# sml2004/CUDA-powered-mesh-handling-and-Iterative-solvers

Measured on NVIDIA B200. Metric: cg_iters_per_s, higher is better.
Workload: dtype f64

## Files before the change

### cuda-powered-mesh-handling-and-iterative-solvers_b200/csrc/dist.cu

```cuda
#include <cstdlib>

#include "spmv_dev.cuh"

namespace femb {

constexpr int MAXP = 16;
constexpr long long SPIN_TIMEOUT_CYCLES = 4000000000ll;

struct SymHeader {
  volatile long long flagA[MAXP];
  volatile long long flagB[MAXP];
  volatile long long flagC[MAXP];
  volatile double redB[MAXP];
  volatile double redC[MAXP];
  volatile double red2[2][4][MAXP];
  double pad[MAXP];
  volatile unsigned long long ll[2][MAXP][8];
  volatile long long flagS[MAXP];
  long long pad2[MAXP];
};
static_assert(sizeof(SymHeader) % 256 == 0, "header keeps p 256-byte aligned");

struct DistState {
  double rs_old, rs_new, pAp, alpha, beta;
// ... 967 lines not shown
    FEMB_CUDA(cudaLaunchCooperativeKernel(kern, dim3(G), dim3(SPMV_THREADS), kargs, 0, s));
    FEMB_CUDA(cudaEventRecord(pev[1], s));
    FEMB_CUDA(cudaMemcpyAsync(hfin, st, sizeof(DistState), cudaMemcpyDeviceToHost, s));
    FEMB_CUDA(cudaStreamSynchronize(s));
    float pms = 0.f;
    cudaEventElapsedTime(&pms, pev[0], pev[1]);
    if (hfin->status == 3 || hfin->stop == 3) {
      set_error("distributed CG: timed out waiting for a peer rank (flag never arrived)");
      return FEMB_ERR_NCCL;
    }
    result_host->iterations = hfin->iterations;
    result_host->status = hfin->status;
    result_host->rs = hfin->rs_new;
    result_host->loop_ms = pms;
    result_host->index_bytes = 4;
    return FEMB_OK;
  }
  if (bptr != nullptr && nnbr > 0 && n_interior > 0 && !getenv("FEMB_DIST_SEPARATE_PUSH")) dist_push_kernel<<<gp, 256, 0, s>>>(pe, send_idx, st);
  cudaGraph_t graph = nullptr;
  cudaGraphExec_t exec = nullptr;
  FEMB_CUDA(cudaStreamBeginCapture(s, cudaStreamCaptureModeThreadLocal));
  const bool folded = bptr != nullptr && nnbr > 0 && n_interior > 0 && !getenv("FEMB_DIST_SEPARATE_PUSH");
  BoundaryPush bp{folded ? bptr : nullptr, bk, boff, n_interior};
  static const bool classic_env = getenv("FEMB_DIST_CLASSIC") != nullptr;
  const bool classic = classic_env && block == 1 && !minv;
  const bool pdl = pdl_enabled() && !classic;
  const long long pin = classic ? 0 : spmv_pin_entries(nnz);
  static const int vec_waves = getenv("FEMB_DIST_VEC_WAVES") ? atoi(getenv("FEMB_DIST_VEC_WAVES")) : 8;
  const int g2m = pdl ? grid_for(n, DV_THREADS, vec_waves) : g2;
  for (int k = 0; k < check_every; ++k) {
// ... 50 lines not shown
  }
  float ms = 0.f;
  if (rc == FEMB_OK) cudaEventElapsedTime(&ms, tev[0], tev[1]);
  cudaGraphExecDestroy(exec);
  cudaGraphDestroy(graph);
  if (rc != FEMB_OK) return rc;
  if (fin->status == 3) {
    set_error("distributed CG: timed out waiting for a peer rank (flag never arrived)");
    return FEMB_ERR_NCCL;
  }
  result_host->iterations = fin->stop ? fin->iterations : max_iter;
  result_host->status = fin->stop ? fin->status : 2;
  result_host->rs = fin->rs_new;
  result_host->loop_ms = ms;
  result_host->index_bytes = 4;
  if (trace && fin->it > 20) {
    static long long h[TRACE_ITERS * 12];
    cudaMemcpy(h, trace, sizeof(h), cudaMemcpyDeviceToHost);
    const int i1 = std::min(fin->it, TRACE_ITERS) - 2;
    double acc[8] = {0, 0, 0, 0, 0, 0, 0, 0};
    for (int i = 10; i < i1; ++i) {
      const long long* t = h + i * 12;
      if (classic) {
        acc[0] += t[1] - t[0];
        acc[1] += t[3] - t[2];
        acc[2] += t[4] - t[3];
        acc[3] += t[6] - t[5];
        acc[4] += t[7] - t[6];
        acc[5] += t[9] - t[8];
        acc[6] += t[10] - t[9];
// ... 22 lines not shown
```

### cuda-powered-mesh-handling-and-iterative-solvers_b200/csrc/krylov.cu

```cuda
#include <cstdlib>

#include "spmv_dev.cuh"

namespace femb {

struct CGState {
  double rs_old, rs_new, pAp, alpha, beta;
  int it, stop, status, iterations;
  unsigned int ticket1, ticket2;
  int fin, fin_status;
};

template <int THREADS>
__device__ __forceinline__ void cg_k1_epilogue_n(double dot, double* __restrict__ partial, CGState* __restrict__ st, double eps, int guards) {
  const double t = block_sum<THREADS>(dot);
  __shared__ bool last;
  if (threadIdx.x == 0) {
    partial[blockIdx.x] = t;
    __threadfence();
    last = atomicAdd(&st->ticket1, 1u) == gridDim.x - 1;
  }
  __syncthreads();
  if (last) {
    __threadfence();
// ... 129 lines not shown
      st ? &st->stop : nullptr, pin, wvec);
  if (st && st->stop) return;
  if (FUSED) {
    if (rvec) cg_k1_epilogue3_n<TMA_THREADS>(dot, extra[0], extra[1], partial, st, eps, guards & 1, tol);
    else cg_k1_epilogue_n<TMA_THREADS>(dot, partial, st, eps, guards & 1);
  }
}

template <bool FUSED>
__global__ void __launch_bounds__(TMA_THREADS) spmv_tma16_kernel(long long n, long long nnz, const int* __restrict__ crow, const int* __restrict__ col,
                                                                 const double* __restrict__ val, const double* __restrict__ x,
                                                                 double* __restrict__ y, const unsigned char* __restrict__ mask,
                                                                 double* __restrict__ partial, CGState* __restrict__ st, double eps, int guards,
                                                                 const double* __restrict__ rvec, double tol, long long pin,
                                                                 const double* __restrict__ wvec, const unsigned short* __restrict__ col16,
                                                                 const unsigned char* __restrict__ tile_ok) {
  pdl_launch_dependents();
  double extra[2] = {0.0, 0.0};
  const double dot = spmv_tma16_rows<TMA16_STAGES, TMA16_CAP>(n, nnz, crow, col, col16, tile_ok, val, x, y, mask, (guards & 2) != 0, FUSED, rvec,
                                                             rvec ? extra : nullptr, st ? &st->stop : nullptr, pin, wvec);
  if (st && st->stop) return;
  if (FUSED) {
    if (rvec) cg_k1_epilogue3_n<TMA_THREADS>(dot, extra[0], extra[1], partial, st, eps, guards & 1, tol);
    else cg_k1_epilogue_n<TMA_THREADS>(dot, partial, st, eps, guards & 1);
  }
}

__global__ void __launch_bounds__(TMA_THREADS) idx16_encode_kernel(long long n, const int* __restrict__ crow, const int* __restrict__ col,
                                                                   unsigned short* __restrict__ col16, unsigned char* __restrict__ tile_ok,
                                                                   int* __restrict__ bad) {
  const long long ntiles = (n + TMA_THREADS - 1) / TMA_THREADS;
  for (long long t = blockIdx.x; t < ntiles; t += gridDim.x) {
    const long long r = t * TMA_THREADS + threadIdx.x;
    bool ok = true;
    if (r < n) {
      const int a = __ldg(crow + r), b = __ldg(crow + r + 1);
      long long prev = r;
      for (int j = a; j < b; ++j) {
        const long long c = __ldg(col + j), d = j == a ? prev - c : c - prev;
        ok = ok && d >= (j == a ? 0 : 1) && d <= 65535;
        col16[j] = (unsigned short)d;
        prev = c;
      }
    }
    ok = __syncthreads_and(ok);
    if (threadIdx.x == 0) {
      tile_ok[t] = ok ? 1 : 0;
      if (!ok) atomicAdd(bad, 1);
    }
  }
}

template <int LR, bool FUSED>
__global__ void __launch_bounds__(TMA_THREADS) spmv_bsr3_tma_kernel(long long nb, long long nnzb, const int* __restrict__ brow,
                                                                    const int* __restrict__ bcol, const double* __restrict__ bval,
                                                                    const double* __restrict__ x, double* __restrict__ y,
                                                                    const unsigned char* __restrict__ mask, double* __restrict__ partial,
                                                                    CGState* __restrict__ st, double eps, int guards,
                                                                    const double* __restrict__ rvec, double tol, const double* __restrict__ wvec) {
  if (st && st->stop) return;
  const double dot = spmv_bsr3_tma_rows<LR, true>(nb, nnzb, brow, bcol, bval, x, y, mask, (guards & 2) != 0, FUSED);
  if (FUSED) cg_k1_epilogue_n<TMA_THREADS>(dot, partial, st, eps, guards & 1);
}

// ... 253 lines not shown
  const double avg = n > 0 ? (double)nnz / (double)n : 1.0;
  static const bool force_vector = getenv("FEMB_SPMV_VECTOR") != nullptr, force_stream = getenv("FEMB_SPMV_STREAM") != nullptr;
  if (force_vector) return -(avg <= 3 ? 2 : avg <= 6 ? 4 : avg <= 24 ? 8 : avg <= 48 ? 16 : 32);
  static const bool force_tma = getenv("FEMB_SPMV_TMA") != nullptr;
  if (!force_stream && !force_tma && avg >= 64.0) return -32;
  if (!force_stream) return 100 + tma_pick_lr(n, nnz);
  for (int lr = 1; lr <= 32; lr *= 2)
    if ((SPMV_THREADS / lr) * avg * 1.25 <= STREAM_CAP) return lr;
  return 32;
}

static thread_local long long nnz_hint = 0;
static thread_local bool pdl_hint = false;
static thread_local long long pin_hint = 0;
static thread_local const unsigned short* col16_hint = nullptr;
static thread_local const unsigned char* tile_ok_hint = nullptr;

template <bool FUSED>
static void launch_spmv(int lanes, int grid, cudaStream_t s, long long n, const int* crow, const int* col, const double* val, const double* x,
                        double* y, const unsigned char* mask, double* partial, CGState* st, double eps, int guards,
                        const double* rvec = nullptr, double tol = 0.0, const double* wvec = nullptr) {
#define FEMB_SPMV_ARGS n, crow, col, val, x, y, mask, partial, st, eps, guards, rvec, tol, wvec
#define FEMB_TMA(LRV)                                                                                                              \
  {                                                                                                                                \
    cudaFuncSetAttribute(spmv_tma_kernel<LRV, FUSED>, cudaFuncAttributeMaxDynamicSharedMemorySize, (int)TMA_SMEM);                 \
    launch_pdl(spmv_tma_kernel<LRV, FUSED>, grid, TMA_THREADS, TMA_SMEM, s, pdl_hint, n, nnz_hint, crow, col, val, x, y, mask, partial, st, eps, \
               guards, rvec, tol, pin_hint, wvec);                                                                               \
  }
#define FEMB_BSR(LRV)                                                                                                              \
  {                                                                                                                                \
    cudaFuncSetAttribute(spmv_bsr3_tma_kernel<LRV, FUSED>, cudaFuncAttributeMaxDynamicSharedMemorySize, (int)BSR_SMEM);            \
// ... 7 lines not shown
    else                                                                                                                           \
      spmv_bsr3_vec_kernel<FUSED, UV, false><<<grid, BSRV_THREADS, 0, s>>>(n / 3, nnz_hint, crow, col, val, x, y, mask, partial, st, eps, guards, rvec, tol, wvec); \
  }
    case 300: FEMB_BSRV(4) break;
    case 301: FEMB_BSRV(2) break;
    case 201: FEMB_BSR(1) break;
    case 202: FEMB_BSR(2) break;
    case 204: FEMB_BSR(4) break;
    case 208: FEMB_BSR(8) break;
    case 216: FEMB_BSR(16) break;
    case 232: FEMB_BSR(32) break;
    case 101:
      if (col16_hint) {
        cudaFuncSetAttribute(spmv_tma16_kernel<FUSED>, cudaFuncAttributeMaxDynamicSharedMemorySize, (int)TMA16_SMEM);
        launch_pdl(spmv_tma16_kernel<FUSED>, grid, TMA_THREADS, TMA16_SMEM, s, pdl_hint, n, nnz_hint, crow, col, val, x, y, mask, partial, st,
                   eps, guards, rvec, tol, pin_hint, wvec, col16_hint, tile_ok_hint);
      } else {
        FEMB_TMA(1)
      }
      break;
    case 102: FEMB_TMA(2) break;
    case 104: FEMB_TMA(4) break;
    case 108: FEMB_TMA(8) break;
    case 116: FEMB_TMA(16) break;
    case 132: FEMB_TMA(32) break;
    case 1: spmv_stream_kernel<1, FUSED><<<grid, SPMV_THREADS, 0, s>>>(FEMB_SPMV_ARGS); break;
    case 2: spmv_stream_kernel<2, FUSED><<<grid, SPMV_THREADS, 0, s>>>(FEMB_SPMV_ARGS); break;
    case 4: spmv_stream_kernel<4, FUSED><<<grid, SPMV_THREADS, 0, s>>>(FEMB_SPMV_ARGS); break;
    case 8: spmv_stream_kernel<8, FUSED><<<grid, SPMV_THREADS, 0, s>>>(FEMB_SPMV_ARGS); break;
    case 16: spmv_stream_kernel<16, FUSED><<<grid, SPMV_THREADS, 0, s>>>(FEMB_SPMV_ARGS); break;
    case 32: spmv_stream_kernel<32, FUSED><<<grid, SPMV_THREADS, 0, s>>>(FEMB_SPMV_ARGS); break;
// ... 76 lines not shown
  SolveCtx* ctx = solve_ctx(as_stream(stream));
  if (!ctx) return FEMB_ERR_CUDA;
  cudaStream_t s = ctx->stream;
  const int guards = minv ? 0 : 1;
  if (minv) eps = 0.0;
  double *r = work, *p = work + n, *Ap = work + 2 * n;
  int lanes[8], g1[8], gmax = 1;
  for (int m = 0; m < nmat; ++m) lanes[m] = pick_lanes(n, mats[m].nnz, mats[m].block);
  static const bool classic_env = getenv("FEMB_CG_CLASSIC") != nullptr;
  const int ll = lanes[nmat - 1];
  static const bool bsr_merged = getenv("FEMB_BSR_MERGED") != nullptr;
  const bool merged = !classic_env && ((ll >= 300 && bsr_merged) || (ll >= 100 && ll < 200) || ll < 0);
  static const bool idx32_env = getenv("FEMB_SPMV_IDX32") != nullptr;
  bool use16 = !idx32_env && merged && nmat == 1 && lanes[0] == 101 && max_iter >= 16;
  const long long ntiles16 = (n + TMA_THREADS - 1) / TMA_THREADS;
  const size_t flags_off = 256, col16_off = flags_off + (((size_t)ntiles16 + 255) & ~(size_t)255);
  if (use16) {
    const size_t need16 = col16_off + 2 * (((size_t)mats[0].nnz + 7) & ~(size_t)7);
    if (ctx->idx16_bytes < need16) {
      if (ctx->graph_exec) cudaGraphExecDestroy(ctx->graph_exec), ctx->graph_exec = nullptr, ctx->graph_key_bytes = 0;
      FEMB_CUDA(cudaStreamSynchronize(s));
      if (ctx->idx16) cudaFree(ctx->idx16);
      ctx->idx16 = nullptr, ctx->idx16_bytes = 0;
      if (cudaMalloc(&ctx->idx16, need16) == cudaSuccess) ctx->idx16_bytes = need16;
      else ctx->idx16 = nullptr, use16 = false, cudaGetLastError();
    }
  }
  if (use16) {
    unsigned char* base16 = static_cast<unsigned char*>(ctx->idx16);
    static_assert(2 * sizeof(CGState) + sizeof(int) <= 512 && 512 + sizeof(int) <= SOLVE_PINNED_BYTES, "pinned status buffer");
    int* bad_host = reinterpret_cast<int*>(static_cast<unsigned char*>(ctx->pinned) + 512);
    FEMB_CUDA(cudaMemsetAsync(base16, 0, sizeof(int), s));
    idx16_encode_kernel<<<(int)std::min<long long>(ntiles16, (long long)SMS * 16), TMA_THREADS, 0, s>>>(
        n, mats[0].crow, mats[0].col, reinterpret_cast<unsigned short*>(base16 + col16_off), base16 + flags_off, reinterpret_cast<int*>(base16));
    FEMB_LAUNCH_CHECK();
    FEMB_CUDA(cudaMemcpyAsync(bad_host, base16, sizeof(int), cudaMemcpyDeviceToHost, s));
    FEMB_CUDA(cudaStreamSynchronize(s));
    use16 = (long long)*bad_host * 100 <= ntiles16;
  }
  const unsigned short* col16 = use16 ? reinterpret_cast<const unsigned short*>(static_cast<unsigned char*>(ctx->idx16) + col16_off) : nullptr;
  const unsigned char* tile_ok = use16 ? static_cast<unsigned char*>(ctx->idx16) + flags_off : nullptr;
  for (int m = 0; m < nmat; ++m) {
    g1[m] = spmv_grid(n, lanes[m], merged && m == nmat - 1);
    if (use16) g1[m] = tma16_grid(n);
    gmax = std::max(gmax, g1[m]);
  }
  const int g2 = grid_for(n, VEC_THREADS, 8);
  static const int vec_waves = getenv("FEMB_VEC_WAVES") ? atoi(getenv("FEMB_VEC_WAVES")) : 8;
  const int g2v = grid_for(n, VEC_THREADS, vec_waves);
  const size_t need = 256 + sizeof(double) * (size_t)std::max(3 * gmax, g2);
  if (ctx->dev_scratch_bytes < need) {
    if (ctx->graph_exec) cudaGraphExecDestroy(ctx->graph_exec), ctx->graph_exec = nullptr, ctx->graph_key_bytes = 0;
    FEMB_CUDA(cudaStreamSynchronize(s));
    if (ctx->dev_scratch) cudaFree(ctx->dev_scratch);
    ctx->dev_scratch = nullptr, ctx->dev_scratch_bytes = 0;
    FEMB_CUDA(cudaMalloc(&ctx->dev_scratch, need + need / 2));
    ctx->dev_scratch_bytes = need + need / 2;
  }
  static_assert(sizeof(CGState) <= 256, "state slot");
  CGState* st = static_cast<CGState*>(ctx->dev_scratch);
  double* partial = reinterpret_cast<double*>(static_cast<unsigned char*>(ctx->dev_scratch) + 256);
  if (mask) cg_mask_kernel<<<g2, VEC_THREADS, 0, s>>>(n, u, mask);
  col16_hint = col16, tile_ok_hint = tile_ok;
  for (int m = 0; m < nmat; ++m)
    nnz_hint = mats[m].nnz, launch_spmv<false>(lanes[m], g1[m], s, n, mats[m].crow, mats[m].col, mats[m].val, u, Ap, nullptr, nullptr, nullptr, 0.0, m ? 2 : 0);
  col16_hint = nullptr, tile_ok_hint = nullptr;
  cg_init_kernel<<<g2, VEC_THREADS, 0, s>>>(n, F, Ap, mask, minv, r, p, partial);
  cg_init_finish<<<1, VEC_THREADS, 0, s>>>(g2, partial, st, max_iter);
  FEMB_LAUNCH_CHECK();
  struct GraphKey {
    long long n;
    int nmat, check_every, max_iter, guards, merged, pdl, lanes[8], g1[8], g2, g2v;
    long long nnz[8];
    const void *crow[8], *col[8], *val[8];
    int block[8];
    const void *mask, *minv, *u, *work, *st, *partial;
    double tol, eps;
    long long pin;
    const void* col16;
  } key;
  memset(&key, 0, sizeof(key));
// ... 8 lines not shown
  static const bool no_cache = getenv("FEMB_NO_GRAPH_CACHE") != nullptr;
  cudaGraph_t graph = nullptr;
  cudaGraphExec_t exec = nullptr;
  if (!no_cache && ctx->graph_exec && ctx->graph_key_bytes == sizeof(key) && memcmp(ctx->graph_key, &key, sizeof(key)) == 0) exec = ctx->graph_exec;
  if (!exec) {
  FEMB_CUDA(cudaStreamBeginCapture(s, cudaStreamCaptureModeThreadLocal));
  for (int k = 0; k < check_every; ++k) {
    for (int m = 0; m + 1 < nmat; ++m)
      nnz_hint = mats[m].nnz, launch_spmv<false>(lanes[m], g1[m], s, n, mats[m].crow, mats[m].col, mats[m].val, p, Ap, nullptr, nullptr, st, 0.0, m ? 2 : 0);
    const int last = nmat - 1;
    nnz_hint = mats[last].nnz;
    if (merged) {
      const bool pdl = pdl_enabled() && nmat == 1 && lanes[last] >= 100 && lanes[last] < 200;
      pdl_hint = pdl && k > 0 && (pdl_mode() & 2);
      pin_hint = pdl ? spmv_pin_entries(mats[last].nnz) : 0;
      col16_hint = col16, tile_ok_hint = tile_ok;
      launch_spmv<true>(lanes[last], g1[last], s, n, mats[last].crow, mats[last].col, mats[last].val, p, Ap, mask, partial, st, eps,
                        guards | (last ? 2 : 0), r, tol, minv);
      pdl_hint = false, pin_hint = 0, col16_hint = nullptr, tile_ok_hint = nullptr;
      launch_pdl(cg_merged_kernel, g2v, VEC_THREADS, 0, s, pdl && (pdl_mode() & 1), n, u, r, p, Ap, minv, partial, st, max_iter, tol);
    } else {
      launch_spmv<true>(lanes[last], g1[last], s, n, mats[last].crow, mats[last].col, mats[last].val, p, Ap, mask, partial, st, eps,
                        guards | (last ? 2 : 0));
      cg_update_kernel<<<g2, VEC_THREADS, 0, s>>>(n, u, r, p, Ap, minv, partial, st, tol, eps, guards, max_iter);
      cg_direction_kernel<<<g2, VEC_THREADS, 0, s>>>(n, r, p, minv, st);
    }
  }
  cudaError_t ce = cudaStreamEndCapture(s, &graph);
  if (ce != cudaSuccess) {
    set_error(std::string("cudaStreamEndCapture: ") + cudaGetErrorString(ce));
    return FEMB_ERR_CUDA;
  }
  FEMB_CUDA(cudaGraphInstantiate(&exec, graph, 0));
  cudaGraphDestroy(graph);
// ... 31 lines not shown
      rc = FEMB_ERR_CUDA;
    }
  }
  float ms = 0.f;
  if (rc == FEMB_OK) cudaEventElapsedTime(&ms, tev[0], tev[1]);
  if (rc != FEMB_OK) {
    cudaGraphExecDestroy(ctx->graph_exec);
    ctx->graph_exec = nullptr, ctx->graph_key_bytes = 0;
    return rc;
  }
  result_host->iterations = fin->stop ? fin->iterations : max_iter;
  result_host->status = fin->stop ? fin->status : 2;
  result_host->rs = fin->rs_new;
  result_host->loop_ms = ms;
  result_host->index_bytes = use16 ? 2 : 4;
  return FEMB_OK;
}

extern "C" int femb_cg_solve(int64_t n, int64_t nnz, const int32_t* crow, const int32_t* col, const double* val, const double* F,
                             const uint8_t* mask, const double* minv, double* u, double* work, double tol, int max_iter, double eps,
                             int check_every, femb_cg_result* result_host, femb_stream stream) {
  FEMB_CHECK_ARG(crow && col && val, "null CSR pointer");
  const CsrRef m{nnz, crow, col, val, 1};
  return cg_solve_impl(n, 1, &m, F, mask, minv, u, work, tol, max_iter, eps, check_every, result_host, stream);
}

extern "C" int femb_spmv_bsr3(int64_t nb, int64_t nnzb, const int32_t* brow, const int32_t* bcol, const double* bval, const double* x,
                              double* y, femb_stream stream) {
  FEMB_CHECK_ARG(nb >= 0 && nnzb >= 0, "nb >= 0, nnzb >= 0");
  if (nb == 0) return FEMB_OK;
// ... 106 lines not shown
    }
  }
  float ms = 0.f;
  if (rc == FEMB_OK) cudaEventElapsedTime(&ms, t0, t1);
  cudaEventDestroy(t0);
  cudaEventDestroy(t1);
  if (rc != FEMB_OK) {
    cudaStreamSynchronize(s);
    return rc;
  }
  result_host->iterations = h.stop ? h.iterations : max_iter;
  result_host->status = h.stop ? h.status : 2;
  result_host->rs = h.rs_new;
  result_host->loop_ms = ms;
  result_host->index_bytes = 0;
  return FEMB_OK;
}
```

### cuda-powered-mesh-handling-and-iterative-solvers_b200/csrc/spmv_dev.cuh

```cuda
#pragma once
#include <cstdlib>

#include "common.cuh"

namespace femb {

constexpr int SPMV_THREADS = 256;
constexpr int STREAM_CAP = 5632;

__device__ __forceinline__ double ld_stream(const double* p) {
  double v;
  asm volatile("ld.global.nc.L1::no_allocate.f64 %0, [%1];" : "=d"(v) : "l"(p));
  return v;
}
__device__ __forceinline__ int ld_stream(const int* p) {
  int v;
  asm volatile("ld.global.nc.L1::no_allocate.s32 %0, [%1];" : "=r"(v) : "l"(p));
  return v;
}
template <bool NC>
__device__ __forceinline__ double ld_x(const double* p) {
  if (NC) return __ldg(p);
  return *p;
}
// ... 296 lines not shown
  }
  return dot;
}

inline int tma_pick_lr(long long n, long long nnz) {
  const double avg = n > 0 ? (double)nnz / (double)n : 1.0;
  for (int lr = 1; lr <= 32; lr *= 2)
    if ((TMA_THREADS / lr) * avg * 1.15 <= TMA_CAP) return lr;
  return 32;
}
inline int tma_grid(long long n, int lr) {
  const long long tiles = (n + TMA_THREADS / lr - 1) / (TMA_THREADS / lr);
  return (int)std::max<long long>(1, std::min<long long>(tiles, (long long)SMS * TMA_CTAS_PER_SM));
}

#ifndef FEMB_TMA16_STAGES
#define FEMB_TMA16_STAGES 2
#endif
#ifndef FEMB_TMA16_CAP
#define FEMB_TMA16_CAP 2176
#endif
#ifndef FEMB_TMA16_CTAS
#define FEMB_TMA16_CTAS 5
#endif
constexpr int TMA16_STAGES = FEMB_TMA16_STAGES, TMA16_CAP = FEMB_TMA16_CAP, TMA16_CTAS_PER_SM = FEMB_TMA16_CTAS;
constexpr size_t TMA16_SMEM = (size_t)TMA16_STAGES * TMA16_CAP * 10;
inline int tma16_grid(long long n) {
  const long long tiles = (n + TMA_THREADS - 1) / TMA_THREADS;
  return (int)std::max<long long>(1, std::min<long long>(tiles, (long long)SMS * TMA16_CTAS_PER_SM));
}

template <int STAGES, int CAP>
__device__ __forceinline__ double spmv_tma16_rows(long long n, long long nnz, const int* __restrict__ crow, const int* __restrict__ col,
                                                  const unsigned short* __restrict__ col16, const unsigned char* __restrict__ tile_ok,
                                                  const double* __restrict__ val, const double* __restrict__ x, double* __restrict__ y,
                                                  const unsigned char* __restrict__ mask, bool accumulate, bool fused,
                                                  const double* __restrict__ rvec, double* extra, const int* stop, long long pin,
                                                  const double* __restrict__ wvec) {
  static_assert(CAP % 8 == 0, "16-byte aligned stages");
  constexpr int R = TMA_THREADS;
  extern __shared__ __align__(128) unsigned char tma_smem[];
  double* vbuf = reinterpret_cast<double*>(tma_smem);
  unsigned short* dbuf = reinterpret_cast<unsigned short*>(tma_smem + sizeof(double) * STAGES * CAP);
  __shared__ unsigned long long full[STAGES];
  __shared__ int base[STAGES];
  const int tid = threadIdx.x;
  const long long ntiles = (n + R - 1) / R;
  const bool use_hint = g_spmv_l2_hint != 0;
  const unsigned long long pol = l2_evict_first_policy(), pol_keep = l2_evict_last_policy();
  if (tid == 0) {
    for (int s = 0; s < STAGES; ++s) mbar_init(&full[s], 1);
    asm volatile("fence.mbarrier_init.release.cluster;" ::: "memory");
  }
  __syncthreads();
  auto bounds = [&](long long k, int& a, int& b, int& ok) {
    const long long t = blockIdx.x + k * gridDim.x;
    a = b = ok = 0;
    if (t < ntiles) a = __ldg(crow + t * R), b = __ldg(crow + min(n, t * R + R)), ok = __ldg(tile_ok + t);
  };
  auto stage_tile = [&](long long k, int a, int b, int ok) {
    if (blockIdx.x + k * gridDim.x >= ntiles) return;
    const int s = (int)(k % STAGES);
    const int a0 = a & ~7, cnt = (b - a0 + 7) & ~7, cntv = (b - a0 + 1) & ~1;
    if (!ok || cnt > CAP || (long long)a0 + cntv > nnz || b == a) {
      base[s] = -1;
      return;
    }
    base[s] = a0;
    asm volatile("fence.proxy.async.shared::cta;" ::: "memory");
    mbar_expect_tx(&full[s], (unsigned)cntv * 8u + (unsigned)cnt * 2u);
    if (use_hint) {
      const unsigned long long pl = (long long)a0 + cntv <= pin ? pol_keep : pol;
      bulk_g2s_hint(vbuf + (size_t)s * CAP, val + a0, (unsigned)cntv * 8u, &full[s], pl);
      bulk_g2s_hint(dbuf + (size_t)s * CAP, col16 + a0, (unsigned)cnt * 2u, &full[s], pl);
    } else {
      bulk_g2s(vbuf + (size_t)s * CAP, val + a0, (unsigned)cntv * 8u, &full[s]);
      bulk_g2s(dbuf + (size_t)s * CAP, col16 + a0, (unsigned)cnt * 2u, &full[s]);
    }
  };
  int na = 0, nb = 0, nok = 0;
  if (tid == 0) {
    for (int k = 0; k < STAGES - 1; ++k) {
      bounds(k, na, nb, nok);
      stage_tile(k, na, nb, nok);
    }
    bounds(STAGES - 1, na, nb, nok);
  }
  double dot = 0.0;
  unsigned phase_bits = 0;
  pdl_wait();
  if (stop) {
    __shared__ int stop_sh;
    if (tid == 0) stop_sh = *(volatile const int*)stop;
    __syncthreads();
    if (stop_sh) {
      for (int k = 0; k < STAGES - 1; ++k)
        if (blockIdx.x + (long long)k * gridDim.x < ntiles && base[k % STAGES] >= 0) mbar_wait(&full[k % STAGES], 0u);
      return 0.0;
    }
  }
  for (long long k = 0;; ++k) {
    const long long t = blockIdx.x + k * gridDim.x;
    if (t >= ntiles) break;
    const int s = (int)(k % STAGES);
    if (tid == 0) {
      stage_tile(k + STAGES - 1, na, nb, nok);
      bounds(k + STAGES, na, nb, nok);
    }
    const long long r = t * R + tid;
    int ra = 0, rb = 0;
    double x_own = 0.0, y_prev = 0.0, r_own = 0.0, w_own = 1.0;
    bool keep = true;
    if (r < n) {
      ra = __ldg(crow + r), rb = __ldg(crow + r + 1);
      if (fused) {
        x_own = __ldg(x + r);
        if (mask) keep = mask[r] != 0;
        if (rvec) r_own = rvec[r];
        if (wvec) w_own = wvec[r];
      }
      if (accumulate) y_prev = y[r];
    }
    __syncthreads();
    const int a0 = base[s];
    double sum = 0.0;
    if (a0 >= 0) {
      mbar_wait(&full[s], (phase_bits >> s) & 1u);
      phase_bits ^= 1u << s;
      const double* vs = vbuf + (size_t)s * CAP - a0;
      const unsigned short* ds = dbuf + (size_t)s * CAP - a0;
      int c = ra < rb ? (int)r - 2 * (int)ds[ra] : 0;
      int j = ra;
      for (; j + 7 < rb; j += 8) {
        double xv[8];
#pragma unroll
        for (int q = 0; q < 8; ++q) c += ds[j + q], xv[q] = __ldg(x + c);
#pragma unroll
        for (int q = 0; q < 8; ++q) sum += vs[j + q] * xv[q];
      }
      {
        double xv[7];
#pragma unroll
        for (int q = 0; q < 7; ++q) {
          if (j + q < rb) c += ds[j + q];
          xv[q] = (j + q < rb) ? __ldg(x + c) : 0.0;
        }
#pragma unroll
        for (int q = 0; q < 7; ++q)
          if (j + q < rb) sum += vs[j + q] * xv[q];
      }
    } else {
      for (int j = ra; j < rb; ++j) sum += ld_stream(val + j) * __ldg(x + ld_stream(col + j));
    }
    if (r < n) {
      if (accumulate) sum += y_prev;
      if (fused) {
        if (!keep) sum = 0.0;
        dot += sum * x_own;
        if (extra) extra[0] += sum * (w_own * r_own), extra[1] += sum * (sum * w_own);
      }
      y[r] = sum;
    }
    __syncthreads();
  }
// ... 160 lines not shown
```

### cuda-powered-mesh-handling-and-iterative-solvers_b200/femb200/_lib.py

```python
from __future__ import annotations

import ctypes as C
import os

_HERE = os.path.dirname(os.path.abspath(__file__))
LIB_PATH = os.path.join(os.path.dirname(_HERE), "libfemb200.so")

c_i32, c_i64, c_f64, c_vp = C.c_int, C.c_int64, C.c_double, C.c_void_p


class CGResult(C.Structure):
    _fields_ = [("iterations", C.c_int32), ("status", C.c_int32), ("rs", C.c_double), ("loop_ms", C.c_double),
                ("index_bytes", C.c_int32)]


APPLY_FN = C.CFUNCTYPE(C.c_int, c_vp, c_vp, c_vp, c_vp)

SIGNATURES = {
    "femb_version": [],
    "femb_elem_volumes": [c_i32, c_vp, c_i32, c_vp, c_i32, c_i64, c_i32, c_vp, c_vp],
    "femb_c3d4": [c_i32, c_vp, c_i32, c_vp, c_i32, c_i64, c_f64, c_f64, c_vp, c_vp, c_vp],
    "femb_solid": [c_i32, c_i32, c_vp, c_i32, c_vp, c_i32, c_i64, C.POINTER(c_f64), c_i32, c_f64, c_f64, c_vp, c_vp],
    "femb_default_points": [c_i32, C.POINTER(c_f64)],
    "femb_mass_points": [c_i32, C.POINTER(c_f64)],
    "femb_solid_stress": [c_i32, c_vp, c_i32, c_vp, c_i32, c_i64, c_vp, C.POINTER(c_f64), c_i32, c_f64, c_f64, c_i32, c_vp, c_vp, c_vp],
    "femb_shape_tables": [c_i32, C.POINTER(c_f64), c_i32, C.POINTER(c_f64), C.POINTER(c_f64)],
    "femb_stress_helper": [c_i32, c_vp, c_i32, c_i64, c_vp, c_vp],
    "femb_node_average": [c_vp, c_vp, c_i32, c_vp, c_vp],
# ... 94 lines not shown
```

### cuda-powered-mesh-handling-and-iterative-solvers_b200/femb200/ops.py

```python
from __future__ import annotations

import collections
import ctypes as C
import os
import weakref

import torch

from . import _lib
from ._lib import CGResult, check, lib

C3D4, C3D6, C3D8, C3D10, C3D15, C3D20, S3, S4 = 4, 6, 8, 10, 15, 20, 103, 104
ENT_TET_FACES, ENT_HEX_FACES, ENT_WEDGE_QUADS, ENT_WEDGE_TRIS, ENT_TRI_EDGES, ENT_QUAD_EDGES = range(6)
_ENT = {ENT_TET_FACES: (4, 3), ENT_HEX_FACES: (6, 4), ENT_WEDGE_QUADS: (3, 4), ENT_WEDGE_TRIS: (2, 3), ENT_TRI_EDGES: (3, 2),
        ENT_QUAD_EDGES: (4, 2)}


def cuda_device(device) -> torch.device:
    d = torch.device(device)
    if d.type != "cuda":
        raise RuntimeError(f"femb200 runs on CUDA devices only (got device={device!r}); there is no CPU fallback")
    if not torch.cuda.is_available():
        raise RuntimeError("femb200 needs a CUDA device (sm_100a); none is visible")
    return d
# ... 517 lines not shown


def cg_solve(crow, col, val, F, mask=None, minv=None, u_init=None, tol=1e-10, max_iter=1000, eps=1e-30, check_every=16):
    dev = val.device
    n = crow.numel() - 1
    Ff = F.to(device=dev, dtype=torch.float64).reshape(-1).contiguous()
    assert Ff.numel() == n, (Ff.numel(), n)
    u = torch.zeros(n, device=dev, dtype=torch.float64) if u_init is None else \
        u_init.to(device=dev, dtype=torch.float64).reshape(-1).clone().contiguous()
    work = torch.empty(4 * n, device=dev, dtype=torch.float64)
    res = CGResult()
    with torch.cuda.device(dev):
        check(lib.femb_cg_solve(n, val.numel(), _p(crow), _p(col), _p(val), _p(Ff), _p(mask), _p(minv), _p(u), _p(work), float(tol),
                                int(max_iter), float(eps), int(check_every), C.byref(res), _stream(dev)), "femb_cg_solve")
    info = {"iterations": res.iterations, "status": STATUS.get(res.status, "?"), "rs": res.rs, "loop_ms": res.loop_ms,
            "index_bytes": res.index_bytes}
    return u.reshape(F.shape), info


def cg_solve_multi(mats, F, mask=None, minv=None, u_init=None, tol=1e-10, max_iter=1000, eps=1e-30, check_every=16):
    dev = mats[0][2].device
    n = mats[0][0].numel() - 1
    Ff = F.to(device=dev, dtype=torch.float64).reshape(-1).contiguous()
    assert Ff.numel() == n and all(m[0].numel() - 1 == n for m in mats)
    u = torch.zeros(n, device=dev, dtype=torch.float64) if u_init is None else \
        u_init.to(device=dev, dtype=torch.float64).reshape(-1).clone().contiguous()
    work = torch.empty(4 * n, device=dev, dtype=torch.float64)
    k = len(mats)
    nnz = (C.c_int64 * k)(*[m[2].numel() for m in mats])
    crow = (C.c_void_p * k)(*[m[0].data_ptr() for m in mats])
    col = (C.c_void_p * k)(*[m[1].data_ptr() for m in mats])
# ... 133 lines not shown
```

### include/femb200.h

```cpp
#ifndef FEMB200_H
#define FEMB200_H

#include <stdint.h>

#ifdef __cplusplus
extern "C" {
#endif

typedef void* femb_stream;

enum {
  FEMB_OK = 0,
  FEMB_ERR_ARG = 1,
  FEMB_ERR_CUDA = 2,
  FEMB_ERR_SINGULAR = 3,
  FEMB_ERR_NCCL = 4,
  FEMB_ERR_UNSUPPORTED = 5
};

const char* femb_last_error(void);
int femb_version(void);


enum { FEMB_C3D4 = 4, FEMB_C3D6 = 6, FEMB_C3D8 = 8, FEMB_C3D10 = 10, FEMB_C3D15 = 15, FEMB_C3D20 = 20, FEMB_S3 = 103, FEMB_S4 = 104 };
// ... 93 lines not shown

int femb_node_average(femb_csr_plan* plan, const void* elem_values, int fp, void* out, femb_stream stream);

int femb_csr_bsr3_convert(int to_bsr, int64_t nb, const int32_t* brow, const double* in, double* out, femb_stream stream);
int femb_spmv_bsr3(int64_t nb, int64_t nnzb, const int32_t* brow, const int32_t* bcol, const double* bval, const double* x, double* y,
                   femb_stream stream);
int femb_bsr3_jacobi(int64_t nb, const int32_t* brow, const int32_t* bcol, const double* bval, const uint8_t* mask, double* minv,
                     femb_stream stream);

typedef struct femb_cg_result {
  int32_t iterations;
  int32_t status;
  double rs;
  double loop_ms;
  int32_t index_bytes;
} femb_cg_result;

int femb_cg_solve(int64_t n, int64_t nnz, const int32_t* crow, const int32_t* col, const double* val, const double* F,
                  const uint8_t* mask, const double* minv, double* u, double* work, double tol, int max_iter, double eps,
                  int check_every, femb_cg_result* result_host, femb_stream stream);

int femb_cg_solve_bsr3(int64_t nb, int64_t nnzb, const int32_t* brow, const int32_t* bcol, const double* bval, const double* F,
                       const uint8_t* mask, const double* minv, double* u, double* work, double tol, int max_iter, double eps,
                       int check_every, femb_cg_result* result_host, femb_stream stream);

int femb_cg_solve_multi(int64_t n, int nmat, const int64_t* nnz_host, const int32_t* const* crow_host,
                        const int32_t* const* col_host, const double* const* val_host, const double* F, const uint8_t* mask,
                        const double* minv, double* u, double* work, double tol, int max_iter, double eps, int check_every,
                        femb_cg_result* result_host, femb_stream stream);

// ... 56 lines not shown
```

Baseline: 2244.

## Stage per-tile x gather windows into shared memory via TMA runs

The index-encode pass now finds, for each row tile, the set of 16-double chunks of x that the tile references. If they fit in a small number of contiguous runs, it rewrites col16 as local offsets into a compacted shared-memory x buffer. The TMA16 SpMV kernel then bulk-copies those x runs into shared memory alongside val/col16 and reads x from smem instead of scattered __ldg gathers. In exchange, staging x costs extra shared memory per stage, which lowers the value CAP and CTAs per SM, and the x runs for the first stages are issued only after the PDL wait.

```diff
diff --git a/cuda-powered-mesh-handling-and-iterative-solvers_b200/csrc/dist.cu b/cuda-powered-mesh-handling-and-iterative-solvers_b200/csrc/dist.cu
--- a/cuda-powered-mesh-handling-and-iterative-solvers_b200/csrc/dist.cu
+++ b/cuda-powered-mesh-handling-and-iterative-solvers_b200/csrc/dist.cu
@@ -1005,6 +1005,7 @@
     result_host->rs = hfin->rs_new;
     result_host->loop_ms = pms;
     result_host->index_bytes = 4;
+  result_host->x_staged_tiles = 0;
     return FEMB_OK;
   }
   if (bptr != nullptr && nnbr > 0 && n_interior > 0 && !getenv("FEMB_DIST_SEPARATE_PUSH")) dist_push_kernel<<<gp, 256, 0, s>>>(pe, send_idx, st);
@@ -1085,6 +1086,7 @@
   result_host->rs = fin->rs_new;
   result_host->loop_ms = ms;
   result_host->index_bytes = 4;
+  result_host->x_staged_tiles = 0;
   if (trace && fin->it > 20) {
     static long long h[TRACE_ITERS * 12];
     cudaMemcpy(h, trace, sizeof(h), cudaMemcpyDeviceToHost);
diff --git a/cuda-powered-mesh-handling-and-iterative-solvers_b200/csrc/krylov.cu b/cuda-powered-mesh-handling-and-iterative-solvers_b200/csrc/krylov.cu
--- a/cuda-powered-mesh-handling-and-iterative-solvers_b200/csrc/krylov.cu
+++ b/cuda-powered-mesh-handling-and-iterative-solvers_b200/csrc/krylov.cu
@@ -1,3 +1,4 @@
+#include <climits>
 #include <cstdlib>
 
 #include "spmv_dev.cuh"
@@ -167,11 +168,12 @@
                                                                  double* __restrict__ partial, CGState* __restrict__ st, double eps, int guards,
                                                                  const double* __restrict__ rvec, double tol, long long pin,
                                                                  const double* __restrict__ wvec, const unsigned short* __restrict__ col16,
-                                                                 const unsigned char* __restrict__ tile_ok) {
+                                                                 const unsigned char* __restrict__ tile_state, const int4* __restrict__ xruns) {
   pdl_launch_dependents();
   double extra[2] = {0.0, 0.0};
-  const double dot = spmv_tma16_rows<TMA16_STAGES, TMA16_CAP>(n, nnz, crow, col, col16, tile_ok, val, x, y, mask, (guards & 2) != 0, FUSED, rvec,
-                                                             rvec ? extra : nullptr, st ? &st->stop : nullptr, pin, wvec);
+  const double dot = spmv_tma16_rows<TMA16_STAGES, TMA16_CAP, TMA16_XCAP>(n, nnz, crow, col, col16, tile_state, xruns, val, x, y, mask,
+                                                                          (guards & 2) != 0, FUSED, rvec, rvec ? extra : nullptr,
+                                                                          st ? &st->stop : nullptr, pin, wvec);
   if (st && st->stop) return;
   if (FUSED) {
     if (rvec) cg_k1_epilogue3_n<TMA_THREADS>(dot, extra[0], extra[1], partial, st, eps, guards & 1, tol);
@@ -179,28 +181,120 @@
   }
 }
 
-__global__ void __launch_bounds__(TMA_THREADS) idx16_encode_kernel(long long n, const int* __restrict__ crow, const int* __restrict__ col,
-                                                                   unsigned short* __restrict__ col16, unsigned char* __restrict__ tile_ok,
-                                                                   int* __restrict__ bad) {
+__device__ __forceinline__ int block_exscan(int v, int* sh, int* total) {
+  constexpr int W = TMA_THREADS / 32;
+  const int lane = threadIdx.x & 31, warp = threadIdx.x >> 5;
+  int inc = v;
+#pragma unroll
+  for (int o = 1; o < 32; o <<= 1) {
+    const int u = __shfl_up_sync(0xffffffffu, inc, o);
+    if (lane >= o) inc += u;
+  }
+  if (lane == 31) sh[warp] = inc;
+  __syncthreads();
+  int below = 0, all = 0;
+#pragma unroll
+  for (int w = 0; w < W; ++w) below += w < warp ? sh[w] : 0, all += sh[w];
+  __syncthreads();
+  *total = all;
+  return below + inc - v;
+}
+
+constexpr int XMAP_WORDS = 1024;
+__global__ void __launch_bounds__(TMA_THREADS) idx16_encode_kernel(long long n, long long nnz, const int* __restrict__ crow, const int* __restrict__ col,
+                                                                   unsigned short* __restrict__ col16, unsigned char* __restrict__ tile_state,
+                                                                   int2* __restrict__ xruns, int* __restrict__ counts, int xsh) {
+  __shared__ unsigned bits[XMAP_WORDS];
+  __shared__ int pre[XMAP_WORDS];
+  __shared__ int red[2][TMA_THREADS / 32];
+  __shared__ int run_first[TMA16_XRUNS], run_slot[TMA16_XRUNS];
+  const int tid = threadIdx.x, lane = tid & 31, warp = tid >> 5;
   const long long ntiles = (n + TMA_THREADS - 1) / TMA_THREADS;
   for (long long t = blockIdx.x; t < ntiles; t += gridDim.x) {
-    const long long r = t * TMA_THREADS + threadIdx.x;
+    const long long r = t * TMA_THREADS + tid;
+    int a = 0, b = 0, lo = INT_MAX, hi = -1;
     bool ok = true;
     if (r < n) {
-      const int a = __ldg(crow + r), b = __ldg(crow + r + 1);
+      a = __ldg(crow + r), b = __ldg(crow + r + 1);
       long long prev = r;
       for (int j = a; j < b; ++j) {
         const long long c = __ldg(col + j), d = j == a ? prev - c : c - prev;
         ok = ok && d >= (j == a ? 0 : 1) && d <= 65535;
-        col16[j] = (unsigned short)d;
         prev = c;
       }
+      if (b > a) lo = (__ldg(col + a) + xsh) >> 4, hi = (__ldg(col + b - 1) + xsh) >> 4;
     }
     ok = __syncthreads_and(ok);
-    if (threadIdx.x == 0) {
-      tile_ok[t] = ok ? 1 : 0;
-      if (!ok) atomicAdd(bad, 1);
-    }
+    int state = ok ? 1 : 0;
+    if (TMA16_XCAP > 0 && ok) {
+      lo = __reduce_min_sync(0xffffffffu, lo), hi = __reduce_max_sync(0xffffffffu, hi);
+      if (lane == 0) red[0][warp] = lo, red[1][warp] = hi;
+      __syncthreads();
+#pragma unroll
+      for (int w = 0; w < TMA_THREADS / 32; ++w) lo = min(lo, red[0][w]), hi = max(hi, red[1][w]);
+      const int ta = __ldg(crow + t * TMA_THREADS), tb = __ldg(crow + min(n, t * TMA_THREADS + TMA_THREADS));
+      const int a0 = ta & ~7, cnt = (tb - a0 + 7) & ~7, cntv = (tb - a0 + 1) & ~1;
+      bool fit = tb > ta && cnt <= TMA16_CAP && (long long)a0 + cntv <= nnz && 16ll * lo - xsh >= 0 && 16ll * hi + 16 - xsh <= n &&
+                 (long long)hi - lo < 32ll * XMAP_WORDS;
+      if (fit) {
+        const int nw = (hi - lo) / 32 + 1;
+        for (int w = tid; w < nw; w += TMA_THREADS) bits[w] = 0;
+        __syncthreads();
+        for (int j = a, last = -1; j < b; ++j) {
+          const int k = ((__ldg(col + j) + xsh) >> 4) - lo;
+          if (k != last) atomicOr(&bits[k >> 5], 1u << (k & 31)), last = k;
+        }
+        __syncthreads();
+        const int per = (nw + TMA_THREADS - 1) / TMA_THREADS, w0 = min(nw, tid * per), w1 = min(nw, w0 + per);
+        int chunks = 0, runs = 0;
+        for (int w = w0; w < w1; ++w) {
+          const unsigned m = bits[w], carry = w ? bits[w - 1] >> 31 : 0u;
+          chunks += __popc(m), runs += __popc(m & ~((m << 1) | carry));
+        }
+        int tot;
+        const int ex = block_exscan(runs << 16 | chunks, red[0], &tot);
+        const int nchunks = tot & 0xffff, nruns = tot >> 16;
+        fit = nchunks * 16 <= TMA16_XCAP && nruns <= TMA16_XRUNS;
+        if (fit) {
+          int slot = ex & 0xffff, run = ex >> 16;
+          for (int w = w0; w < w1; ++w) {
+            const unsigned m = bits[w], carry = w ? bits[w - 1] >> 31 : 0u;
+            pre[w] = slot;
+            for (unsigned s = m & ~((m << 1) | carry); s; s &= s - 1, ++run) {
+              const int bit = __ffs(s) - 1;
+              run_first[run] = 16 * (lo + 32 * w + bit) - xsh, run_slot[run] = slot + __popc(m & ((1u << bit) - 1));
+            }
+            slot += __popc(m);
+          }
+          __syncthreads();
+          if (tid < TMA16_XRUNS) {
+            int2 v = make_int2(0, 0);
+            if (tid < nruns) v = make_int2(run_first[tid], 16 * ((tid + 1 < nruns ? run_slot[tid + 1] : nchunks) - run_slot[tid]));
+            xruns[t * TMA16_XRUNS + tid] = v;
+          }
+          state = 2;
+        }
+      }
+    }
+    if (r < n) {
+      long long prev = r;
+      for (int j = a; j < b; ++j) {
+        const int c = __ldg(col + j);
+        if (state == 2) {
+          const int k = ((c + xsh) >> 4) - lo;
+          col16[j] = (unsigned short)(16 * (pre[k >> 5] + __popc(bits[k >> 5] & ((1u << (k & 31)) - 1))) + ((c + xsh) & 15));
+        } else {
+          col16[j] = (unsigned short)(j == a ? prev - c : c - prev);
+        }
+        prev = c;
+      }
+    }
+    if (tid == 0) {
+      tile_state[t] = (unsigned char)state;
+      if (!ok) atomicAdd(counts, 1);
+      if (state == 2) atomicAdd(counts + 1, 1);
+    }
+    __syncthreads();
   }
 }
 
@@ -484,7 +578,8 @@
 static thread_local bool pdl_hint = false;
 static thread_local long long pin_hint = 0;
 static thread_local const unsigned short* col16_hint = nullptr;
-static thread_local const unsigned char* tile_ok_hint = nullptr;
+static thread_local const unsigned char* tile_state_hint = nullptr;
+static thread_local const int4* xruns_hint = nullptr;
 
 template <bool FUSED>
 static void launch_spmv(int lanes, int grid, cudaStream_t s, long long n, const int* crow, const int* col, const double* val, const double* x,
@@ -522,7 +617,7 @@
       if (col16_hint) {
         cudaFuncSetAttribute(spmv_tma16_kernel<FUSED>, cudaFuncAttributeMaxDynamicSharedMemorySize, (int)TMA16_SMEM);
         launch_pdl(spmv_tma16_kernel<FUSED>, grid, TMA_THREADS, TMA16_SMEM, s, pdl_hint, n, nnz_hint, crow, col, val, x, y, mask, partial, st,
-                   eps, guards, rvec, tol, pin_hint, wvec, col16_hint, tile_ok_hint);
+                   eps, guards, rvec, tol, pin_hint, wvec, col16_hint, tile_state_hint, xruns_hint);
       } else {
         FEMB_TMA(1)
       }
@@ -629,7 +724,10 @@
   static const bool idx32_env = getenv("FEMB_SPMV_IDX32") != nullptr;
   bool use16 = !idx32_env && merged && nmat == 1 && lanes[0] == 101 && max_iter >= 16;
   const long long ntiles16 = (n + TMA_THREADS - 1) / TMA_THREADS;
-  const size_t flags_off = 256, col16_off = flags_off + (((size_t)ntiles16 + 255) & ~(size_t)255);
+  const size_t flags_off = 256, runs_off = flags_off + (((size_t)ntiles16 + 255) & ~(size_t)255);
+  const size_t col16_off = runs_off + ((TMA16_XCAP ? (size_t)ntiles16 * TMA16_XRUNS * sizeof(int2) + 255 : 0) & ~(size_t)255);
+  const int xsh = (int)((reinterpret_cast<uintptr_t>(work + n) >> 3) & 1);
+  int xstaged = 0;
   if (use16) {
     const size_t need16 = col16_off + 2 * (((size_t)mats[0].nnz + 7) & ~(size_t)7);
     if (ctx->idx16_bytes < need16) {
@@ -643,18 +741,22 @@
   }
   if (use16) {
     unsigned char* base16 = static_cast<unsigned char*>(ctx->idx16);
-    static_assert(2 * sizeof(CGState) + sizeof(int) <= 512 && 512 + sizeof(int) <= SOLVE_PINNED_BYTES, "pinned status buffer");
-    int* bad_host = reinterpret_cast<int*>(static_cast<unsigned char*>(ctx->pinned) + 512);
-    FEMB_CUDA(cudaMemsetAsync(base16, 0, sizeof(int), s));
+    static_assert(2 * sizeof(CGState) <= 512 && 512 + 2 * sizeof(int) <= SOLVE_PINNED_BYTES, "pinned status buffer");
+    int* counts_host = reinterpret_cast<int*>(static_cast<unsigned char*>(ctx->pinned) + 512);
+    FEMB_CUDA(cudaMemsetAsync(base16, 0, 2 * sizeof(int), s));
     idx16_encode_kernel<<<(int)std::min<long long>(ntiles16, (long long)SMS * 16), TMA_THREADS, 0, s>>>(
-        n, mats[0].crow, mats[0].col, reinterpret_cast<unsigned short*>(base16 + col16_off), base16 + flags_off, reinterpret_cast<int*>(base16));
+        n, mats[0].nnz, mats[0].crow, mats[0].col, reinterpret_cast<unsigned short*>(base16 + col16_off), base16 + flags_off,
+        reinterpret_cast<int2*>(base16 + runs_off), reinterpret_cast<int*>(base16), xsh);
     FEMB_LAUNCH_CHECK();
-    FEMB_CUDA(cudaMemcpyAsync(bad_host, base16, sizeof(int), cudaMemcpyDeviceToHost, s));
+    FEMB_CUDA(cudaMemcpyAsync(counts_host, base16, 2 * sizeof(int), cudaMemcpyDeviceToHost, s));
     FEMB_CUDA(cudaStreamSynchronize(s));
-    use16 = (long long)*bad_host * 100 <= ntiles16;
-  }
-  const unsigned short* col16 = use16 ? reinterpret_cast<const unsigned short*>(static_cast<unsigned char*>(ctx->idx16) + col16_off) : nullptr;
-  const unsigned char* tile_ok = use16 ? static_cast<unsigned char*>(ctx->idx16) + flags_off : nullptr;
+    use16 = (long long)counts_host[0] * 100 <= ntiles16;
+    xstaged = use16 ? counts_host[1] : 0;
+  }
+  unsigned char* idx16 = static_cast<unsigned char*>(ctx->idx16);
+  const unsigned short* col16 = use16 ? reinterpret_cast<const unsigned short*>(idx16 + col16_off) : nullptr;
+  const unsigned char* tile_state = use16 ? idx16 + flags_off : nullptr;
+  const int4* xruns = use16 && TMA16_XCAP ? reinterpret_cast<const int4*>(idx16 + runs_off) : nullptr;
   for (int m = 0; m < nmat; ++m) {
     g1[m] = spmv_grid(n, lanes[m], merged && m == nmat - 1);
     if (use16) g1[m] = tma16_grid(n);
@@ -676,10 +778,10 @@
   CGState* st = static_cast<CGState*>(ctx->dev_scratch);
   double* partial = reinterpret_cast<double*>(static_cast<unsigned char*>(ctx->dev_scratch) + 256);
   if (mask) cg_mask_kernel<<<g2, VEC_THREADS, 0, s>>>(n, u, mask);
-  col16_hint = col16, tile_ok_hint = tile_ok;
+  if (!xstaged || (int)((reinterpret_cast<uintptr_t>(u) >> 3) & 1) == xsh) col16_hint = col16, tile_state_hint = tile_state, xruns_hint = xruns;
   for (int m = 0; m < nmat; ++m)
     nnz_hint = mats[m].nnz, launch_spmv<false>(lanes[m], g1[m], s, n, mats[m].crow, mats[m].col, mats[m].val, u, Ap, nullptr, nullptr, nullptr, 0.0, m ? 2 : 0);
-  col16_hint = nullptr, tile_ok_hint = nullptr;
+  col16_hint = nullptr, tile_state_hint = nullptr, xruns_hint = nullptr;
   cg_init_kernel<<<g2, VEC_THREADS, 0, s>>>(n, F, Ap, mask, minv, r, p, partial);
   cg_init_finish<<<1, VEC_THREADS, 0, s>>>(g2, partial, st, max_iter);
   FEMB_LAUNCH_CHECK();
@@ -718,10 +820,10 @@
       const bool pdl = pdl_enabled() && nmat == 1 && lanes[last] >= 100 && lanes[last] < 200;
       pdl_hint = pdl && k > 0 && (pdl_mode() & 2);
       pin_hint = pdl ? spmv_pin_entries(mats[last].nnz) : 0;
-      col16_hint = col16, tile_ok_hint = tile_ok;
+      col16_hint = col16, tile_state_hint = tile_state, xruns_hint = xruns;
       launch_spmv<true>(lanes[last], g1[last], s, n, mats[last].crow, mats[last].col, mats[last].val, p, Ap, mask, partial, st, eps,
                         guards | (last ? 2 : 0), r, tol, minv);
-      pdl_hint = false, pin_hint = 0, col16_hint = nullptr, tile_ok_hint = nullptr;
+      pdl_hint = false, pin_hint = 0, col16_hint = nullptr, tile_state_hint = nullptr, xruns_hint = nullptr;
       launch_pdl(cg_merged_kernel, g2v, VEC_THREADS, 0, s, pdl && (pdl_mode() & 1), n, u, r, p, Ap, minv, partial, st, max_iter, tol);
     } else {
       launch_spmv<true>(lanes[last], g1[last], s, n, mats[last].crow, mats[last].col, mats[last].val, p, Ap, mask, partial, st, eps,
@@ -783,6 +885,7 @@
   result_host->rs = fin->rs_new;
   result_host->loop_ms = ms;
   result_host->index_bytes = use16 ? 2 : 4;
+  result_host->x_staged_tiles = xstaged;
   return FEMB_OK;
 }
 
@@ -919,5 +1022,6 @@
   result_host->rs = h.rs_new;
   result_host->loop_ms = ms;
   result_host->index_bytes = 0;
+  result_host->x_staged_tiles = 0;
   return FEMB_OK;
 }
diff --git a/cuda-powered-mesh-handling-and-iterative-solvers_b200/csrc/spmv_dev.cuh b/cuda-powered-mesh-handling-and-iterative-solvers_b200/csrc/spmv_dev.cuh
--- a/cuda-powered-mesh-handling-and-iterative-solvers_b200/csrc/spmv_dev.cuh
+++ b/cuda-powered-mesh-handling-and-iterative-solvers_b200/csrc/spmv_dev.cuh
@@ -334,36 +334,42 @@
   return (int)std::max<long long>(1, std::min<long long>(tiles, (long long)SMS * TMA_CTAS_PER_SM));
 }
 
+#ifndef FEMB_TMA16_XCAP
+#define FEMB_TMA16_XCAP 1024
+#endif
 #ifndef FEMB_TMA16_STAGES
 #define FEMB_TMA16_STAGES 2
 #endif
 #ifndef FEMB_TMA16_CAP
-#define FEMB_TMA16_CAP 2176
+#define FEMB_TMA16_CAP (FEMB_TMA16_XCAP ? 1984 : 2176)
 #endif
 #ifndef FEMB_TMA16_CTAS
-#define FEMB_TMA16_CTAS 5
+#define FEMB_TMA16_CTAS (FEMB_TMA16_XCAP ? 4 : 5)
 #endif
 constexpr int TMA16_STAGES = FEMB_TMA16_STAGES, TMA16_CAP = FEMB_TMA16_CAP, TMA16_CTAS_PER_SM = FEMB_TMA16_CTAS;
-constexpr size_t TMA16_SMEM = (size_t)TMA16_STAGES * TMA16_CAP * 10;
+constexpr int TMA16_XCAP = FEMB_TMA16_XCAP, TMA16_XRUNS = 8;
+constexpr size_t TMA16_SMEM = (size_t)TMA16_STAGES * ((size_t)TMA16_CAP * 10 + (size_t)TMA16_XCAP * 8);
 inline int tma16_grid(long long n) {
   const long long tiles = (n + TMA_THREADS - 1) / TMA_THREADS;
   return (int)std::max<long long>(1, std::min<long long>(tiles, (long long)SMS * TMA16_CTAS_PER_SM));
 }
 
-template <int STAGES, int CAP>
+template <int STAGES, int CAP, int XCAP>
 __device__ __forceinline__ double spmv_tma16_rows(long long n, long long nnz, const int* __restrict__ crow, const int* __restrict__ col,
-                                                  const unsigned short* __restrict__ col16, const unsigned char* __restrict__ tile_ok,
-                                                  const double* __restrict__ val, const double* __restrict__ x, double* __restrict__ y,
-                                                  const unsigned char* __restrict__ mask, bool accumulate, bool fused,
-                                                  const double* __restrict__ rvec, double* extra, const int* stop, long long pin,
-                                                  const double* __restrict__ wvec) {
-  static_assert(CAP % 8 == 0, "16-byte aligned stages");
-  constexpr int R = TMA_THREADS;
+                                                  const unsigned short* __restrict__ col16, const unsigned char* __restrict__ tile_state,
+                                                  const int4* __restrict__ xruns, const double* __restrict__ val,
+                                                  const double* __restrict__ x, double* __restrict__ y, const unsigned char* __restrict__ mask,
+                                                  bool accumulate, bool fused, const double* __restrict__ rvec, double* extra, const int* stop,
+                                                  long long pin, const double* __restrict__ wvec) {
+  static_assert(CAP % 8 == 0 && XCAP % 16 == 0, "16-byte aligned stages");
+  constexpr int R = TMA_THREADS, XQ = TMA16_XRUNS / 2;
   extern __shared__ __align__(128) unsigned char tma_smem[];
   double* vbuf = reinterpret_cast<double*>(tma_smem);
-  unsigned short* dbuf = reinterpret_cast<unsigned short*>(tma_smem + sizeof(double) * STAGES * CAP);
+  double* xbuf = vbuf + (size_t)STAGES * CAP;
+  unsigned short* dbuf = reinterpret_cast<unsigned short*>(xbuf + (size_t)STAGES * XCAP);
   __shared__ unsigned long long full[STAGES];
   __shared__ int base[STAGES];
+  __shared__ bool xst[STAGES];
   const int tid = threadIdx.x;
   const long long ntiles = (n + R - 1) / R;
   const bool use_hint = g_spmv_l2_hint != 0;
@@ -373,22 +379,46 @@
     asm volatile("fence.mbarrier_init.release.cluster;" ::: "memory");
   }
   __syncthreads();
-  auto bounds = [&](long long k, int& a, int& b, int& ok) {
+  auto bounds = [&](long long k, int& a, int& b, int& st, int4(&xr)[XQ]) {
     const long long t = blockIdx.x + k * gridDim.x;
-    a = b = ok = 0;
-    if (t < ntiles) a = __ldg(crow + t * R), b = __ldg(crow + min(n, t * R + R)), ok = __ldg(tile_ok + t);
+    a = b = st = 0;
+    if (t < ntiles) {
+      a = __ldg(crow + t * R), b = __ldg(crow + min(n, t * R + R)), st = __ldg(tile_state + t);
+      if constexpr (XCAP > 0) {
+#pragma unroll
+        for (int q = 0; q < XQ; ++q) xr[q] = __ldg(xruns + t * XQ + q);
+      }
+    }
   };
-  auto stage_tile = [&](long long k, int a, int b, int ok) {
+  auto stage_x = [&](int s, const int4(&xr)[XQ]) {
+    double* xs = xbuf + (size_t)s * XCAP;
+    int slot = 0;
+#pragma unroll
+    for (int q = 0; q < XQ; ++q) {
+      if (xr[q].y) bulk_g2s(xs + slot, x + xr[q].x, (unsigned)xr[q].y * 8u, &full[s]);
+      slot += xr[q].y;
+      if (xr[q].w) bulk_g2s(xs + slot, x + xr[q].z, (unsigned)xr[q].w * 8u, &full[s]);
+      slot += xr[q].w;
+    }
+  };
+  auto stage_tile = [&](long long k, int a, int b, int st, const int4(&xr)[XQ], bool with_x) {
     if (blockIdx.x + k * gridDim.x >= ntiles) return;
     const int s = (int)(k % STAGES);
     const int a0 = a & ~7, cnt = (b - a0 + 7) & ~7, cntv = (b - a0 + 1) & ~1;
-    if (!ok || cnt > CAP || (long long)a0 + cntv > nnz || b == a) {
+    if (!st || cnt > CAP || (long long)a0 + cntv > nnz || b == a) {
       base[s] = -1;
       return;
     }
     base[s] = a0;
+    const bool sx = XCAP > 0 && st == 2;
+    xst[s] = sx;
+    unsigned xbytes = 0;
+    if (sx) {
+#pragma unroll
+      for (int q = 0; q < XQ; ++q) xbytes += (unsigned)(xr[q].y + xr[q].w) * 8u;
+    }
     asm volatile("fence.proxy.async.shared::cta;" ::: "memory");
-    mbar_expect_tx(&full[s], (unsigned)cntv * 8u + (unsigned)cnt * 2u);
+    mbar_expect_tx(&full[s], (unsigned)cntv * 8u + (unsigned)cnt * 2u + xbytes);
     if (use_hint) {
       const unsigned long long pl = (long long)a0 + cntv <= pin ? pol_keep : pol;
       bulk_g2s_hint(vbuf + (size_t)s * CAP, val + a0, (unsigned)cntv * 8u, &full[s], pl);
@@ -397,18 +427,30 @@
       bulk_g2s(vbuf + (size_t)s * CAP, val + a0, (unsigned)cntv * 8u, &full[s]);
       bulk_g2s(dbuf + (size_t)s * CAP, col16 + a0, (unsigned)cnt * 2u, &full[s]);
     }
+    if (sx && with_x) stage_x(s, xr);
   };
-  int na = 0, nb = 0, nok = 0;
+  int na = 0, nb = 0, nst = 0;
+  int4 nxr[XQ] = {}, pxr[STAGES - 1][XQ] = {};
   if (tid == 0) {
+#pragma unroll
     for (int k = 0; k < STAGES - 1; ++k) {
-      bounds(k, na, nb, nok);
-      stage_tile(k, na, nb, nok);
-    }
-    bounds(STAGES - 1, na, nb, nok);
+      bounds(k, na, nb, nst, nxr);
+      stage_tile(k, na, nb, nst, nxr, false);
+#pragma unroll
+      for (int q = 0; q < XQ; ++q) pxr[k][q] = nxr[q];
+    }
+    bounds(STAGES - 1, na, nb, nst, nxr);
   }
   double dot = 0.0;
   unsigned phase_bits = 0;
   pdl_wait();
+  if constexpr (XCAP > 0) {
+    if (tid == 0) {
+#pragma unroll
+      for (int k = 0; k < STAGES - 1; ++k)
+        if (blockIdx.x + (long long)k * gridDim.x < ntiles && base[k % STAGES] >= 0 && xst[k % STAGES]) stage_x(k % STAGES, pxr[k]);
+    }
+  }
   if (stop) {
     __shared__ int stop_sh;
     if (tid == 0) stop_sh = *(volatile const int*)stop;
@@ -424,8 +466,8 @@
     if (t >= ntiles) break;
     const int s = (int)(k % STAGES);
     if (tid == 0) {
-      stage_tile(k + STAGES - 1, na, nb, nok);
-      bounds(k + STAGES, na, nb, nok);
+      stage_tile(k + STAGES - 1, na, nb, nst, nxr, true);
+      bounds(k + STAGES, na, nb, nst, nxr);
     }
     const long long r = t * R + tid;
     int ra = 0, rb = 0;
@@ -449,25 +491,43 @@
       phase_bits ^= 1u << s;
       const double* vs = vbuf + (size_t)s * CAP - a0;
       const unsigned short* ds = dbuf + (size_t)s * CAP - a0;
-      int c = ra < rb ? (int)r - 2 * (int)ds[ra] : 0;
-      int j = ra;
-      for (; j + 7 < rb; j += 8) {
-        double xv[8];
-#pragma unroll
-        for (int q = 0; q < 8; ++q) c += ds[j + q], xv[q] = __ldg(x + c);
-#pragma unroll
-        for (int q = 0; q < 8; ++q) sum += vs[j + q] * xv[q];
-      }
-      {
+      if (XCAP > 0 && xst[s]) {
+        const double* xs = xbuf + (size_t)s * XCAP;
+        int j = ra;
+        for (; j + 7 < rb; j += 8) {
+          double xv[8];
+#pragma unroll
+          for (int q = 0; q < 8; ++q) xv[q] = xs[ds[j + q]];
+#pragma unroll
+          for (int q = 0; q < 8; ++q) sum += vs[j + q] * xv[q];
+        }
         double xv[7];
 #pragma unroll
-        for (int q = 0; q < 7; ++q) {
-          if (j + q < rb) c += ds[j + q];
-          xv[q] = (j + q < rb) ? __ldg(x + c) : 0.0;
-        }
+        for (int q = 0; q < 7; ++q) xv[q] = (j + q < rb) ? xs[ds[j + q]] : 0.0;
 #pragma unroll
         for (int q = 0; q < 7; ++q)
           if (j + q < rb) sum += vs[j + q] * xv[q];
+      } else {
+        int c = ra < rb ? (int)r - 2 * (int)ds[ra] : 0;
+        int j = ra;
+        for (; j + 7 < rb; j += 8) {
+          double xv[8];
+#pragma unroll
+          for (int q = 0; q < 8; ++q) c += ds[j + q], xv[q] = __ldg(x + c);
+#pragma unroll
+          for (int q = 0; q < 8; ++q) sum += vs[j + q] * xv[q];
+        }
+        {
+          double xv[7];
+#pragma unroll
+          for (int q = 0; q < 7; ++q) {
+            if (j + q < rb) c += ds[j + q];
+            xv[q] = (j + q < rb) ? __ldg(x + c) : 0.0;
+          }
+#pragma unroll
+          for (int q = 0; q < 7; ++q)
+            if (j + q < rb) sum += vs[j + q] * xv[q];
+        }
       }
     } else {
       for (int j = ra; j < rb; ++j) sum += ld_stream(val + j) * __ldg(x + ld_stream(col + j));
diff --git a/cuda-powered-mesh-handling-and-iterative-solvers_b200/femb200/_lib.py b/cuda-powered-mesh-handling-and-iterative-solvers_b200/femb200/_lib.py
--- a/cuda-powered-mesh-handling-and-iterative-solvers_b200/femb200/_lib.py
+++ b/cuda-powered-mesh-handling-and-iterative-solvers_b200/femb200/_lib.py
@@ -11,7 +11,7 @@
 
 class CGResult(C.Structure):
     _fields_ = [("iterations", C.c_int32), ("status", C.c_int32), ("rs", C.c_double), ("loop_ms", C.c_double),
-                ("index_bytes", C.c_int32)]
+                ("index_bytes", C.c_int32), ("x_staged_tiles", C.c_int32)]
 
 
 APPLY_FN = C.CFUNCTYPE(C.c_int, c_vp, c_vp, c_vp, c_vp)
diff --git a/cuda-powered-mesh-handling-and-iterative-solvers_b200/femb200/ops.py b/cuda-powered-mesh-handling-and-iterative-solvers_b200/femb200/ops.py
--- a/cuda-powered-mesh-handling-and-iterative-solvers_b200/femb200/ops.py
+++ b/cuda-powered-mesh-handling-and-iterative-solvers_b200/femb200/ops.py
@@ -555,7 +555,7 @@
         check(lib.femb_cg_solve(n, val.numel(), _p(crow), _p(col), _p(val), _p(Ff), _p(mask), _p(minv), _p(u), _p(work), float(tol),
                                 int(max_iter), float(eps), int(check_every), C.byref(res), _stream(dev)), "femb_cg_solve")
     info = {"iterations": res.iterations, "status": STATUS.get(res.status, "?"), "rs": res.rs, "loop_ms": res.loop_ms,
-            "index_bytes": res.index_bytes}
+            "index_bytes": res.index_bytes, "x_staged_tiles": res.x_staged_tiles}
     return u.reshape(F.shape), info
 
 
diff --git a/include/femb200.h b/include/femb200.h
--- a/include/femb200.h
+++ b/include/femb200.h
@@ -131,6 +131,7 @@
   double rs;
   double loop_ms;
   int32_t index_bytes;
+  int32_t x_staged_tiles;
 } femb_cg_result;
 
 int femb_cg_solve(int64_t n, int64_t nnz, const int32_t* crow, const int32_t* col, const double* val, const double* F,
```

Result: slower. 2190, median of 6 (-2.4%).
